# rahulgaur104/ideal-ballooning-solver

Measured on AMD Instinct MI355X. Metric: field-line eigenvalue solves/sec (N_zeta=512), higher is better.
Workload: dtype f64; 1 GPU; configs[1] D3D-shape: 16 surfaces x 8 alpha x 8 theta0 = 1024 solves/step/GPU, N_zeta=512 (513 points), geometry-fed scan with fused per-surface argmax (one launch); nonconverged=0, ranks_in_collective=1

## Files before the change

### ideal-ballooning-solver_amd/csrc/ibs_group.hpp

```cpp
#pragma once
#include "ibs_wave.hpp"

namespace ibs {

template <int P>
struct Grp {
  static_assert(P == 16 || P == 32 || P == 64, "group size");
  static constexpr int G = 64 / P;

  template <typename T>
  __device__ __forceinline__ static T bcast_last(T v, int lane) {
    if constexpr (P == 64) return readlane_t(v, 63);
    else if constexpr (P == 32) { const T a = readlane_t(v, 31), b = readlane_t(v, 63); return lane < 32 ? a : b; }
    else return dpp_t<0x15F, 0xF>(v, v);
  }
  __device__ __forceinline__ static int bcast_last_i(int v, int lane) {
    if constexpr (P == 64) return readlane_i(v, 63);
    else if constexpr (P == 32) { const int a = readlane_i(v, 31), b = readlane_i(v, 63); return lane < 32 ? a : b; }
    else return dpp_i<0x15F, 0xF>(v, v);
  }
  template <typename T>
  __device__ __forceinline__ static T sum(T v, int lane) {
    v += dppz_t<0x111, 0xF>(v);
    v += dppz_t<0x112, 0xF>(v);
// ... 56 lines not shown
    const int l16 = lane & 15, row = lane >> 4;
    { const M2<T> F = dpp_fetch<T, 0x101, 0xF>(Q); if (l16 < 15) Q = mul<T, false>(Q, F); }
    { const M2<T> F = dpp_fetch<T, 0x102, 0xF>(Q); if (l16 < 14) Q = mul<T, true>(Q, F); }
    { const M2<T> F = dpp_fetch<T, 0x104, 0xF>(Q); if (l16 < 12) Q = mul<T, false>(Q, F); }
    { const M2<T> F = dpp_fetch<T, 0x108, 0xF>(Q); if (l16 < 8) Q = mul<T, true>(Q, F); }
    if constexpr (P >= 32) {
      const M2<T> t16 = lane_bcast(Q, 16), t48 = lane_bcast(Q, 48);
      M2<T> F;
      F.a = row == 0 ? t16.a : t48.a; F.b = row == 0 ? t16.b : t48.b;
      F.c = row == 0 ? t16.c : t48.c; F.d = row == 0 ? t16.d : t48.d; F.e = row == 0 ? t16.e : t48.e;
      if ((row & 1) == 0) Q = mul<T, P == 32>(Q, F);
    }
    if constexpr (P == 64) { const M2<T> F = lane_bcast(Q, 32); if (row < 2) Q = mul<T, true>(Q, F); }
    return Q;
  }
};

template <typename T, int M, int P>
struct GroupSolver {
  using GP = Grp<P>;
  static constexpr int G = 64 / P;
  T D[M], Ph[M];
  T kap, ikap;
  bool has_last;
  int lane, lg, gid;
  T sig_vec;
  T zw[M];
  T u0_in;
  T zu_m1, zw_p1;
  int Eu, Ew;
  T lo, hi, normA;
  T trial_rho, trial_del;
  T trial_mrg;
  T shoot_m; int shoot_e;
  T fu, fw;
  int thr;

  __device__ __forceinline__ static int rows_start(int lg_, int n) {
    const int rem = n - P * (M - 1);
    return lg_ * (M - 1) + (lg_ < rem ? lg_ : rem);
  }

  template <class Src, bool TRIAL = false>
  __device__ __forceinline__ bool setup(const Src& src, int N, T h) {
    lane = threadIdx.x & 63;
    lg = lane & (P - 1);
    gid = lane / P;
    const int n = N - 2;
    const int rem = n - P * (M - 1);
    has_last = lg < rem;
    const int a = rows_start(lg, n);
    const T ih2 = T(1) / (h * h);
    T sc = T(1);
    const T g0 = src.g(a);
    T gcur = src.g(a + 1);
    T e_lo = T(0.5) * (g0 + gcur) * ih2;
    T vhi = -T(1e300), vlo = -T(1e300), vna = T(0), sum_c = T(0), sum_f = T(0);
    bool bad = !(g0 > T(0)) || !(gcur > T(0));
    const T e_first = e_lo;
    T ts_prev = T(0), ts_cur = T(0), two_cd = T(0), tA = T(0), tB = T(0), tC = T(0);
    if constexpr (TRIAL) {
      const T dl = T(3.14159265358979323846) / T(N - 1);
      T s0, c0, sd, cd;
      trial_sincos(T(a) * dl, s0, c0);
      trial_sincos(dl, sd, cd);
      ts_prev = s0; ts_cur = xfma(s0, cd, c0 * sd); two_cd = T(2) * cd;
    }
#pragma unroll
    for (int i = 0; i < M; ++i) {
      const bool act = (i < M - 1) || has_last;
      if (act) {
        const int j = a + i + 1;
        const T gnext = src.g(j + 1);
        bad = bad || !(gnext > T(0));
        const T e_hi = T(0.5) * (gcur + gnext) * ih2;
        const T cj = src.c(j), fj = src.f(j);
        const T d = cj - (e_lo + e_hi);
        const T s2 = sc * sc;
        D[i] = d * s2; Ph[i] = fj * s2;
        const T rf = fast_rcp(fj);
        if constexpr (TRIAL) {
          const T ts_next = xfma(two_cd, ts_cur, -ts_prev);
          const T Tx = xfma(e_lo, ts_prev, xfma(d, ts_cur, e_hi * ts_next));
          tA = xfma(ts_cur, Tx, tA); tB = xfma(fj * ts_cur, ts_cur, tB); tC = xfma(Tx * rf, Tx, tC);
          ts_prev = ts_cur; ts_cur = ts_next;
        }
        vhi = xmax(vhi, cj * rf);
        vlo = xmax(vlo, d * rf);
        vna = xmax(vna, (xabs(d) + e_lo + e_hi) * rf);
        sum_c += cj; sum_f += fj;
        bad = bad || !(fj > T(0)) || !(e_hi > T(0)) || !finite_of(cj);
        sc = fast_rcp(e_hi * sc);
        gcur = gnext; e_lo = e_hi;
      } else {
        D[i] = T(0); Ph[i] = T(0);
      }
    }
    kap = sc; ikap = fast_rcp(sc);
    bad = bad || !(e_first > T(0));
    const T ends = GP::sum((lg == 0 ? e_first : T(0)) + (lg == P - 1 ? e_lo : T(0)), lane);
    const T sc_all = GP::sum(sum_c, lane), sf_all = GP::sum(sum_f, lane);
    normA = GP::max(vna, lane);
    hi = GP::max(vhi, lane);
    lo = xmax(GP::max(vlo, lane), (sc_all - ends) / sf_all);
    hi += T(8) * Eps<T>::v * normA;
    lo -= T(8) * Eps<T>::v * normA;
    if constexpr (TRIAL) {
      const T A = GP::sum(tA, lane), B = GP::sum(tB, lane), C = GP::sum(tC, lane);
      const T rho = A / B;
      trial_rho = rho;
      trial_del = approx_sqrt(xmax(xfma(-rho, A, C), T(0)) / B);
    } else {
      trial_rho = T(0); trial_del = T(-1);
    }
    trial_mrg = T(8 + N / 2) * Eps<T>::v * normA;
    chk_slack = T(N < 256 ? 2 * N : 512) * Eps<T>::v * normA;
    return GP::sum_i(bad ? 1 : 0, lane) != 0;
  }

  __device__ __forceinline__ void trial_guess(bool take, T& guess, T& width, bool& warm) {
    const bool use = take && finite_of(trial_rho) && trial_del > T(0) && trial_del < T(0.25) * (hi - lo);
    lo = use ? xmax(lo, trial_rho - trial_mrg) : lo;
    guess = use ? trial_rho : guess;
    width = use ? T(0.25) * trial_del : width;
    warm = use ? true : warm;
  }

  template <bool STORE = true>
// ... 108 lines not shown
      const T a_um1 = readlane_t(zum_b, sLk), a_wp1 = readlane_t(zwp_b, sLk);
      const int a_ik = readlane_i(bi, sLk), a_Eu = readlane_i(Eu, sLk), a_Ew = readlane_i(Ew, sLk);
      zu_k = mine ? a_zu : zu_k; zw_k = mine ? a_zw : zw_k; t_k = mine ? a_t : t_k;
      um1 = mine ? a_um1 : um1; wp1 = mine ? a_wp1 : wp1;
      ik = mine ? a_ik : ik; Euk = mine ? a_Eu : Euk; Ewk = mine ? a_Ew : Ewk;
    }
    const T uw = zu_k * zw_k;
    const T num = xfma(um1, zw_k, xfma(t_k, uw, wp1 * zu_k));
    int du = Eu - Euk, dw = Ew - Ewk;
    du = du > 1000 ? 1000 : (du < -2000 ? -2000 : du);
    dw = dw > 1000 ? 1000 : (dw < -2000 ? -2000 : dw);
    fu = xldexp(fast_rcp(zu_k), du);
    fw = xldexp(fast_rcp(zw_k), dw);
    thr = (lane < Lk) ? M : ((lane > Lk) ? -1 : ik);
    T acc = T(0);
    static_assert(M + 2 <= 32, "sign word");
    unsigned su = sign_word(zu_m1) >> 31, sw = 0;
    {
      T zc = u0_in, zp = zu_m1;
#pragma unroll
      for (int i = 0; i < M; ++i) {
        const T t = xfma(-sig, Ph[i], D[i]);
        const bool act = (i < M - 1) || has_last;
        const T xu = zc * fu, xw = zw[i] * fw;
        const T x = (i <= thr) ? xu : xw;
        if (act) acc = xfma(Ph[i] * x, x, acc);
        if constexpr (CNT) {
          su = (unsigned)__builtin_amdgcn_alignbit(su, sign_word(zc), 31);
          sw = (unsigned)__builtin_amdgcn_alignbit(sw, sign_word(zw[i]), 31);
        }
        const T zn = xfma(-t, zc, -zp);
        if (act) { zp = zc; zc = zn; }
      }
    }
    if constexpr (CNT) {
      const int last = has_last ? M - 1 : M - 2;
      const int iu = thr < last ? thr : last;
      const unsigned mu = iu >= 0 ? (((1u << (iu + 1)) - 1u) << (M - 1 - iu)) : 0u;
      const int iw = thr > 0 ? thr : 0;
      const unsigned mw = iw <= last ? (((1u << (last - iw + 1)) - 1u) << (M - last)) : 0u;
      const unsigned sw2 = (sw << 1) | (sign_word(zw_p1) >> 31);
      extra_above = GP::sum_i(__builtin_popcount((su ^ (su >> 1)) & mu) + __builtin_popcount((sw2 ^ (sw2 << 1)) & mw), lane);
    }
    sig_vec = sig;
    const T tot = GP::sum(acc, lane);
    return sig + num * fast_rcp(uw * tot);
  }

  template <class Src>
  __device__ __forceinline__ void assemble(const Src& src, int N, T h, T (&x)[M]) {
    const int a = rows_start(lg, N - 2);
    const T ih2 = T(1) / (h * h);
    T sc = T(1);
    T gcur = src.g(a + 1);
    T zc = u0_in, zp = zu_m1;
#pragma unroll
    for (int i = 0; i < M; ++i) {
      const bool act = (i < M - 1) || has_last;
      const T xu = sc * zc * fu, xw = sc * zw[i] * fw;
      x[i] = act ? ((i <= thr) ? xu : xw) : T(0);
      if (act) {
        const T gnext = src.g(a + i + 2);
        sc = fast_rcp(T(0.5) * (gcur + gnext) * ih2 * sc);
        gcur = gnext;
        const T zn = xfma(-xfma(-sig_vec, Ph[i], D[i]), zc, -zp);
        zp = zc; zc = zn;
      }
    }
  }

  bool suspect, closed;
  T rho_last;
  __device__ __forceinline__ int why() const {
    const T tol = T(64) * Eps<T>::v * normA, rho = rho_last;
    const T dist = xmax(xmax(lo - rho, rho - hi), T(0));
    int bk = dist > T(0) ? expo_of(dist) - expo_of(tol) + 8 : 0;
    bk = finite_of(rho) ? (bk < 1 ? (dist > T(0) ? 1 : 0) : (bk > 63 ? 63 : bk)) : 63;
    return closed ? (bk | (extra_above != 0 ? 64 : 0)) : 0;
  }
  T chk_slack;
  template <bool CHK = false>
  __device__ __forceinline__ T solve(bool bad, int& iters_out, int& status_out, bool warm = false, T guess = T(0),
                                     T width = T(0)) {
    using WS = WaveSolver<T, M>;
    using Pt = typename WS::Pt;
    const T tol = (sizeof(T) == 8 ? T(64) : T(8)) * Eps<T>::v * normA;
    const bool warm_ok = warm && finite_of(guess) && width > T(0) && guess + width < hi && guess + width > lo;
    bool expand = warm_ok, try_below = warm_ok;
    T wstep = T(4) * width;
    const T g_below = guess - width;
    T sig = warm_ok ? guess + width : T(0.5) * (lo + hi), sig_prev = sig, lam = hi;
    T off_up = tol, off_dn = tol, rho_trust = hi;
    int aimed = 0, it = 0, lg_prev = 0;
    bool lo1 = false, hi_f = false, old_ok = false, was_interp = false, conv = false;
    Pt Plo{lo, T(0), 0}, Phi{hi, T(0), 0}, Pold{hi, T(0), 0};
    bool done = bad;
    constexpr int kMaxIt = 200;
    int guard = 0;
    auto sel = [](bool c, const Pt& a, const Pt& b) { return Pt{c ? a.x : b.x, c ? a.m : b.m, c ? a.e : b.e}; };
    while (__any(!done) && guard < kMaxIt) {
      ++guard;
      const int C = sweep_fwd<true>(sig);
      const bool act = !done;
      it += act ? 1 : 0;
      const Pt cur{sig, shoot_m, shoot_e};
      const bool uh = act && C == 0, ul = act && C != 0;
      const bool t1 = uh && hi_f, t2 = ul && lo1;
      Pold = sel(t1, Phi, sel(t2, Plo, Pold)); old_ok = old_ok || t1 || t2;
      hi = uh ? sig : hi; Phi = sel(uh, cur, Phi); hi_f = hi_f || uh;
      lo = ul ? sig : lo; Plo = sel(ul, cur, Plo); lo1 = ul ? (C == 1) : lo1;
      const T prevstep = xabs(sig - sig_prev);
      sig_prev = sig;
      const int e_now = expo_of(shoot_m);
      const int red = lg_prev - (e_now < -(1 << 27) ? e_now : shoot_e + e_now);
      conv = was_interp ? (red >= 4) : (aimed != 0 ? conv : false);
      const bool force_bis = was_interp && red < 1;
      const bool cert = aimed != 0;
// ... 75 lines not shown
```

### ideal-ballooning-solver_amd/csrc/ibs_kernels.hip

```cpp
#include "ibs_wave.hpp"
#include "ibs_launch.hpp"
#include "ibs_refine.hpp"
#include <type_traits>

#ifndef IBS_M
#error "compile with -DIBS_M=<rows per lane>"
#endif
#ifndef IBS_DIRECT_MIN_M
#define IBS_DIRECT_MIN_M 9
#endif
#ifndef IBS_F32LAM_DIRECT_MIN_M
#define IBS_F32LAM_DIRECT_MIN_M 3
#endif

namespace ibs {

template <typename T>
struct SrcGCF {
  static constexpr bool kHasGh = false;
  const T* gs; const T* cs; const T* fs;
  __device__ __forceinline__ T g(int j) const { return gs[lpos(j)]; }
  __device__ __forceinline__ T c(int j) const { return cs[lpos(j)]; }
  __device__ __forceinline__ T f(int j) const { return fs[lpos(j)]; }
  __device__ __forceinline__ void gcf(int j, T& g_, T& c_, T& f_) const { const int q = lpos(j); g_ = gs[q]; c_ = cs[q]; f_ = fs[q]; }
// ... 139 lines not shown
      src.gcf(jc, g_, c_, f_);
    }
    y0 += c_ * X2 - g_ * dX2;
    y1 = xfma(f_, X2, y1);
    if constexpr (!std::is_same<Tan, NoTangent>::value) {
      T ga, ca, fa;
      tan->at(jc, ga, ca, fa);
      ac = xfma(ca, X2, ac); ag = xfma(ga, dX2, ag); af = xfma(fa, X2, af);
    }
    if (X_out && in) X_out[sys * N + j] = (TO)X;
    if (dX_out && in) dX_out[sys * N + j] = (TO)dX;
  }
  IBS_PROBE_AT(14);
  y0 = wave_sum(y0); y1 = wave_sum(y1);
  const T gam = y0 / y1;
  if constexpr (HF) {
    if (do_hf) {
      hc = wave_sum(hc); hg = wave_sum(hg); hf = wave_sum(hf);
      const T jac = hc / y1 - hg / y1 - gam * hf / y1;
      if (lane == 0) dth0_out[sys] = (TO)jac;
    }
  }
  if constexpr (!std::is_same<Tan, NoTangent>::value) {
    ac = wave_sum(ac); ag = wave_sum(ag); af = wave_sum(af);
    const T jac = ac / y1 - ag / y1 - gam * af / y1;
    if (lane == 0 && dalpha_out) dalpha_out[sys] = (TO)jac;
  }
  if (lane == 0) {
    if (gam_out) __hip_atomic_store(gam_out + sys, (TO)gam, __ATOMIC_RELAXED, __HIP_MEMORY_SCOPE_AGENT);
    if (lam_out) lam_out[sys] = (TO)lam;
    if (info_out) info_out[sys] = inf.iters | (inf.status << 16);
  }
}

template <typename T, class Src, bool WT>
__device__ __forceinline__ void simpson_point(const Src& src, int j, T w, T X, T dX, T& y0, T& y1, T& hc, T& hg, T& hf) {
  const T X2 = w * (X * X), dX2 = w * (dX * dX);
  T g_, c_, f_;
  if constexpr (WT) {
    T gt, ct, ft;
    src.gcf_with_tangent(j, g_, c_, f_, gt, ct, ft);
    hc = xfma(ct, X2, hc); hg = xfma(gt, dX2, hg); hf = xfma(ft, X2, hf);
  } else {
    src.gcf(j, g_, c_, f_);
  }
  y0 += c_ * X2 - g_ * dX2;
  y1 = xfma(f_, X2, y1);
}

template <typename T, class Src, bool WT>
__device__ __forceinline__ void simpson_point_carried(const Src& src, int j, T a1, T d_, T c_, T f_, T w, T X, T dX, T& y0, T& y1,
                                                      T& hc, T& hg, T& hf) {
  const T X2 = w * (X * X), dX2 = w * (dX * dX);
  asm volatile("" : "+v"(d_));
  const T g_ = a1 * d_;
  if constexpr (WT) {
    T gt, ct, ft;
    src.tangent(j, a1, gt, ct, ft);
    hc = xfma(ct, X2, hc); hg = xfma(gt, dX2, hg); hf = xfma(ft, X2, hf);
  }
  y0 += c_ * X2 - g_ * dX2;
  y1 = xfma(f_, X2, y1);
}

template <typename T, int M, class Src, bool HF, int PASSES = 1, typename TO = T, bool RES = false>
__device__ __forceinline__ void finish_chunk(WaveSolver<T, M, RES>& ws, Src& src, int N, T h, T* Xs, T lam,
                                             const SolveInfo& inf, long sys, typename TypeId<TO>::type* lam_out,
                                             typename TypeId<TO>::type* gam_out, typename TypeId<TO>::type* X_out,
                                             typename TypeId<TO>::type* dX_out, typename TypeId<TO>::type* dth0_out,
                                             int* info_out, const T* gh = nullptr) {
  static_assert(M >= 3, "the halo exchange takes two rows from each neighbour lane");
  const int lane = ws.lane;
  const int n = N - 2;
  const bool hl = ws.has_last;
  T x[M];
  ws.assemble(src, gh, N, h, x);
  T m = T(0);
#pragma unroll
  for (int i = 0; i < M; ++i) m = xmax(m, xabs(x[i]));
  m = uniform(wave_max(m));
  const T rm = T(1) / m;
#pragma unroll
  for (int i = 0; i < M; ++i) x[i] *= rm;
  int a = WaveSolver<T, M>::rows_start(lane, n);
  asm volatile("" : "+v"(a));
  const T lastv = hl ? x[M - 1] : x[M - 2], last2 = hl ? x[M - 2] : x[M - 3];
  const T xp1 = dpp_t<0x130, 0xF>(T(0), x[0]), xp2 = dpp_t<0x130, 0xF>(T(0), x[1]);
  T xe[M + 4];
  xe[0] = dpp_t<0x138, 0xF>(T(0), last2); xe[1] = dpp_t<0x138, 0xF>(T(0), lastv);
#pragma unroll
  for (int i = 0; i < M - 1; ++i) xe[i + 2] = x[i];
  xe[M + 1] = hl ? x[M - 1] : xp1; xe[M + 2] = hl ? xp1 : xp2; xe[M + 3] = xp2;
  IBS_PROBE_AT(13);
  T ih;
  if constexpr (RES) ih = ws.rr.ih; else ih = T(1) / h;
  const T A_in = (T(2) / T(3)) * ih, B_in = -ih / T(12), A_e1 = T(0.5) * ih, A_e0 = T(2) * ih, B_e0 = T(-0.5) * ih;
  bool do_hf = false;
  if constexpr (HF) do_hf = dth0_out != nullptr;
  T y0 = T(0), y1 = T(0), hc = T(0), hg = T(0), hf = T(0);
  const T w_even = ((a + 1) & 1) ? T(4) : T(2), w_odd = ((a + 1) & 1) ? T(2) : T(4);
  const int i_end = (lane == kWave - 1) ? (hl ? M - 1 : M - 2) : -1;
  const T dX_end = xfma(A_e0, lane == 0 ? x[0] : -lastv, B_e0 * (lane == 0 ? x[1] : -last2));
  auto all_points = [&](auto with_tangent) {
    if (lane == 0 || lane == kWave - 1)
      simpson_point<T, Src, HF && decltype(with_tangent)::value>(src, lane == 0 ? 0 : N - 1, T(1), T(0), dX_end, y0, y1, hc, hg, hf);
#pragma unroll
    for (int i = 0; i < M; ++i) {
// ... 1545 lines not shown
```

### ideal-ballooning-solver_amd/csrc/ibs_kernels_group.hip

```cpp
#include <type_traits>
#include "ibs_group.hpp"
#include "ibs_launch.hpp"

#if !defined(IBS_M) || !defined(IBS_P)
#error "compile with -DIBS_P=<lanes per system> -DIBS_M=<rows per lane>"
#endif

namespace ibs {

template <typename T, typename TI = T>
struct SrcGlobal {
  static constexpr bool kHasGh = false;
  const TI* gs; const TI* cs; const TI* fs;
  __device__ __forceinline__ T g(int j) const { return (T)gs[j]; }
  __device__ __forceinline__ T c(int j) const { return (T)cs[j]; }
  __device__ __forceinline__ T f(int j) const { return (T)fs[j]; }
};

template <typename T>
struct SrcGeoG {
  static constexpr bool kHasGh = false;
  const T* A1; const T* A3; const T* C0; const T* C1; const T* G0; const T* G1; const T* G2;
  T th0, two_th0, th0sq;
  __device__ __forceinline__ T gd(int j) const { const int q = lpos(j); return G0[q] + two_th0 * G1[q] + th0sq * G2[q]; }
  __device__ __forceinline__ T g(int j) const { return A1[lpos(j)] * gd(j); }
  __device__ __forceinline__ T c(int j) const { const int q = lpos(j); return C0[q] + th0 * C1[q]; }
  __device__ __forceinline__ T f(int j) const { return A3[lpos(j)] * gd(j); }
  __device__ __forceinline__ T gdp(int j) const { const int q = lpos(j); return T(2) * G1[q] + two_th0 * G2[q]; }
  __device__ __forceinline__ T g_t(int j) const { return A1[lpos(j)] * gdp(j); }
  __device__ __forceinline__ T c_t(int j) const { return C1[lpos(j)]; }
  __device__ __forceinline__ T f_t(int j) const { return A3[lpos(j)] * gdp(j); }
};

template <typename T, class Src, bool WT>
__device__ __forceinline__ void simpson_point_g(const Src& src, int j, T w, T X, T dX, T& y0, T& y1, T& hc, T& hg, T& hf) {
  const T X2 = w * (X * X), dX2 = w * (dX * dX);
  y0 += src.c(j) * X2 - src.g(j) * dX2;
  y1 = xfma(src.f(j), X2, y1);
  if constexpr (WT) { hc = xfma(src.c_t(j), X2, hc); hg = xfma(src.g_t(j), dX2, hg); hf = xfma(src.f_t(j), X2, hf); }
}

template <typename T, int M, int P, class Src, bool HF, typename TO = T>
__device__ __forceinline__ void finish_chunk_g(GroupSolver<T, M, P>& ws, const Src& src, int N, T h, T* Xs, T lam,
                                               int iters, int status, long sys, bool valid, TO* lam_out, TO* gam_out,
                                               TO* X_out, TO* dX_out, TO* dth0_out, int* info_out) {
  static_assert(M >= 3, "the halo exchange takes two rows from each neighbour lane");
  using GP = Grp<P>;
  const int lane = ws.lane, lg = ws.lg;
  const int n = N - 2;
  const bool hl = ws.has_last, first = lg == 0, last = lg == P - 1;

  T x[M];
  ws.assemble(src, N, h, x);
  T m = T(0);
#pragma unroll
  for (int i = 0; i < M; ++i) m = xmax(m, xabs(x[i]));
  m = GP::max(m, lane);
  const T rm = T(1) / m;
#pragma unroll
  for (int i = 0; i < M; ++i) x[i] *= rm;
  int a = GroupSolver<T, M, P>::rows_start(lg, n);
  asm volatile("" : "+v"(a));
  const T lastv = hl ? x[M - 1] : x[M - 2], last2 = hl ? x[M - 2] : x[M - 3];
  const T sp1 = dpp_t<0x130, 0xF>(T(0), x[0]), sp2 = dpp_t<0x130, 0xF>(T(0), x[1]);
  const T sm2 = dpp_t<0x138, 0xF>(T(0), last2), sm1 = dpp_t<0x138, 0xF>(T(0), lastv);
  const T xp1 = last ? T(0) : sp1, xp2 = last ? T(0) : sp2;
  T xe[M + 4];
  xe[0] = first ? T(0) : sm2; xe[1] = first ? T(0) : sm1;
#pragma unroll
  for (int i = 0; i < M - 1; ++i) xe[i + 2] = x[i];
  xe[M + 1] = hl ? x[M - 1] : xp1; xe[M + 2] = hl ? xp1 : xp2; xe[M + 3] = xp2;
  const T ih = T(1) / h;
  const T A_in = (T(2) / T(3)) * ih, B_in = -ih / T(12), A_e1 = T(0.5) * ih, A_e0 = T(2) * ih, B_e0 = T(-0.5) * ih;
  bool do_hf = false;
  if constexpr (HF) do_hf = dth0_out != nullptr;
  T y0 = T(0), y1 = T(0), hc = T(0), hg = T(0), hf = T(0);
  const T w_even = ((a + 1) & 1) ? T(4) : T(2), w_odd = ((a + 1) & 1) ? T(2) : T(4);
  const int i_end = last ? (hl ? M - 1 : M - 2) : -1;
// ... 310 lines not shown
```

### ideal-ballooning-solver_amd/csrc/ibs_wave.hpp

```cpp
#pragma once
#include <hip/hip_runtime.h>
#include <type_traits>
#include "ibs_sweep_count.hpp"

namespace ibs {

constexpr int kWave = 64;

#ifdef IBS_TRACE_ALL
__device__ double ibs_trace_all[404];
#endif
#ifdef IBS_PROBE
__device__ long long ibs_probe_buf[(16 + 4) * 4096];
#define IBS_PROBE_SLOT(k) ibs_probe_buf[(k) < 16 ? (blockIdx.x * 4 + (threadIdx.x >> 6)) * 16 + (k) \
                                                 : 16 * 4096 + (blockIdx.x * 4 + (threadIdx.x >> 6)) * 4 + ((k) - 16)]
#define IBS_PROBE_NOW() wall_clock64()
#define IBS_PROBE_PUT(k, t) do { if ((threadIdx.x & 63) == 0 && blockIdx.x < 1024 && threadIdx.x < 256) IBS_PROBE_SLOT(k) = (t); } while (0)
#define IBS_PROBE_AT(k) IBS_PROBE_PUT(k, wall_clock64())
#else
#define IBS_PROBE_AT(k) do {} while (0)
#define IBS_PROBE_NOW() 0LL
#define IBS_PROBE_PUT(k, t) do { (void)(t); } while (0)
#endif



__device__ __forceinline__ int fexp(double x) { return __builtin_amdgcn_frexp_exp(x); }
__device__ __forceinline__ int fexp(float x) { return __builtin_amdgcn_frexp_expf(x); }
__device__ __forceinline__ double xldexp(double x, int e) { return __builtin_ldexp(x, e); }
__device__ __forceinline__ float xldexp(float x, int e) { return __builtin_ldexpf(x, e); }
__device__ __forceinline__ double xfma(double a, double b, double c) { return __builtin_fma(a, b, c); }
__device__ __forceinline__ float xfma(float a, float b, float c) { return __builtin_fmaf(a, b, c); }
__device__ __forceinline__ double xabs(double a) { return __builtin_fabs(a); }
__device__ __forceinline__ float xabs(float a) { return __builtin_fabsf(a); }
__device__ __forceinline__ double xmax(double a, double b) { return __builtin_fmax(a, b); }
__device__ __forceinline__ float xmax(float a, float b) { return __builtin_fmaxf(a, b); }
__device__ __forceinline__ double xmin(double a, double b) { return __builtin_fmin(a, b); }
__device__ __forceinline__ float xmin(float a, float b) { return __builtin_fminf(a, b); }
__device__ __forceinline__ bool signbit_of(double a) { return __double2hiint(a) < 0; }
__device__ __forceinline__ bool signbit_of(float a) { return __float_as_int(a) < 0; }
__device__ __forceinline__ bool sign_differs(double a, double b) {
  int x = __double2hiint(a) ^ __double2hiint(b);
  asm("" : "+v"(x));
  return x < 0;
}
__device__ __forceinline__ bool sign_differs(float a, float b) { return (__float_as_int(a) ^ __float_as_int(b)) < 0; }
__device__ __forceinline__ unsigned sign_word(double a) { return (unsigned)__double2hiint(a); }
__device__ __forceinline__ unsigned sign_word(float a) { return (unsigned)__float_as_int(a); }
__device__ __forceinline__ bool finite_of(double a) { return xabs(a) <= 1.7976931348623157e308; }
__device__ __forceinline__ bool finite_of(float a) { return xabs(a) <= 3.4028234e38f; }

__device__ __forceinline__ double fast_rcp(double x) {
  double r = __builtin_amdgcn_rcp(x);
  r = __builtin_fma(__builtin_fma(-x, r, 1.0), r, r);
  r = __builtin_fma(__builtin_fma(-x, r, 1.0), r, r);
  return r;
// ... 317 lines not shown
}

template <typename T, class CountF>
__device__ __forceinline__ bool multisect(CountF&& count, T lo, T hi, T normA, T stop_eps, int lane, T& lam, int& passes) {
  const T epsA = Eps<T>::v * normA;
  bool ok = false;
  passes = 0;
  while (passes < 24) {
    ++passes;
    const T w = hi - lo;
    const T sig = lane == kWave - 1 ? hi : xfma(T(lane) * T(1.0 / 63.0), w, lo);
    const int cnt = count(sig);
    const unsigned long long m = __builtin_amdgcn_ballot_w64(cnt >= 1);
    if (!(m & 1ull)) { hi = lo; lo = lo - T(64) * w; continue; }
    const int top = 63 - __builtin_clzll(m);
    if (top == kWave - 1) { lo = hi; hi = hi + T(64) * w; continue; }
    lo = readlane_t(sig, top); hi = readlane_t(sig, top + 1);
    if (!(hi - lo > stop_eps * epsA)) { ok = true; break; }
  }
  lam = T(0.5) * (lo + hi);
  return ok;
}
template <typename T, class CountF>
__device__ __forceinline__ bool multisect_k(CountF&& count, int k, T lo, T hi, T normA, T stop_eps, int lane, T& lam, int& passes) {
  const T epsA = Eps<T>::v * normA;
  bool ok = false;
  passes = 0;
  while (passes < 24) {
    ++passes;
    const T w = hi - lo;
    const T sig = lane == kWave - 1 ? hi : xfma(T(lane) * T(1.0 / 63.0), w, lo);
    const int cnt = count(sig);
    const unsigned long long m = __builtin_amdgcn_ballot_w64(cnt >= k);
    if (!(m & 1ull)) { hi = lo; lo = lo - T(64) * w; continue; }
    const int top = 63 - __builtin_clzll(m);
    if (top == kWave - 1) { lo = hi; hi = hi + T(64) * w; continue; }
    lo = readlane_t(sig, top); hi = readlane_t(sig, top + 1);
    if (!(hi - lo > stop_eps * epsA)) { ok = true; break; }
  }
  lam = T(0.5) * (lo + hi);
  return ok;
}
template <typename T, class Src>
__device__ __forceinline__ bool multisect_division(const Src& src, int N, T h, T lo, T hi, T normA, int lane, T& lam, int& passes) {
  const T ih2 = T(1) / (h * h);
  return multisect<T>([&](T sig) { return count_above_div<T, Src>(src, N, ih2, sig); }, lo, hi, normA, T(2), lane, lam, passes);
}
template <typename T, class Src>
__device__ __forceinline__ bool reclose_division(const Src& src, int N, T h, T center, T normA, int lane, T& lam, int& passes) {
  const T epsA = Eps<T>::v * normA;
  return multisect_division<T, Src>(src, N, h, center - T(2048) * epsA, center + T(2048) * epsA, normA, lane, lam, passes);
}

struct SolveInfo {
  int iters;
  int status;
};

template <typename T, int M, bool RES>
struct ResidentRows {};
template <typename T, int M>
struct ResidentRows<T, M, true> {
  T a1[M], d[M], c[M], f[M], zu[M];
  T ih2, ih;
  unsigned own;
};

template <typename T, int M, bool RES = false>
struct WaveSolver {
  ResidentRows<T, M, RES> rr;
  T D[M], Ph[M];
  T kap, ikap;
  bool has_last;
  int lane;
  T zw[M];
  T u0_in, zu_m1;
  T zw_p1;
  int Eu, Ew;
  T sig_vec;
  T lo, hi, normA;
  T trial_rho, trial_del;
  T trial_mrg;
  T shoot_m; int shoot_e;

  static constexpr int kSetupRows = 4;
  __device__ __forceinline__ static int rows_start(int lane, int n) {
    const int rem = n - kWave * (M - 1);
    return lane * (M - 1) + (lane < rem ? lane : rem);
  }

  template <class Src, bool TRIAL = false>
  __device__ __forceinline__ bool setup(const Src& src, int N, T h) {
    lane = threadIdx.x & (kWave - 1);
    const int n = N - 2;
    const int rem = n - kWave * (M - 1);
    has_last = lane < rem;
    if constexpr (RES) rr.own = sweep_count_mask(M, has_last, lane == kWave - 1);
    const int a = rows_start(lane, n);
    T ih2;
    if constexpr (RES) ih2 = rr.ih2; else ih2 = T(1) / (h * h);
    T sc = T(1);
    T gcur = T(0);
    T e_lo;
    bool bad = false;
    if constexpr (Src::kHasGh) {
      e_lo = src.gh(a) * ih2;
      bad = !(src.g(a) > T(0));
    } else {
      const T g0 = src.g(a);
      gcur = src.g(a + 1);
      e_lo = T(0.5) * (g0 + gcur) * ih2;
      bad = !(g0 > T(0)) || !(gcur > T(0));
    }
    T vhi = -T(1e300), vlo = -T(1e300), vna = T(0), sum_c = T(0), sum_f = T(0);
    const T e_first = e_lo;
    T ts_prev = T(0), ts_cur = T(0), two_cd = T(0), tA = T(0), tB = T(0), tC = T(0);
    if constexpr (TRIAL) {
      const T dl = T(3.14159265358979323846) / T(N - 1);
      T s0, c0, sd, cd;
      trial_sincos(T(a) * dl, s0, c0);
      trial_sincos(dl, sd, cd);
      ts_prev = s0; ts_cur = xfma(s0, cd, c0 * sd); two_cd = T(2) * cd;
    }
#pragma unroll
    for (int i = 0; i < M; ++i) {
      const bool act = (i < M - 1) || has_last;
      if (act) {
        const int j = a + i + 1;
        T gnext = T(0), e_hi;
        if constexpr (Src::kHasGh) { e_hi = src.gh(j) * ih2; bad = bad || !(src.g(j + 1) > T(0)); }
        else { gnext = src.g(j + 1); e_hi = T(0.5) * (gcur + gnext) * ih2; bad = bad || !(gnext > T(0)); }
        const T cj = src.c(j), fj = src.f(j);
        const T d = cj - (e_lo + e_hi);
        const T s2 = sc * sc;
        D[i] = d * s2; Ph[i] = fj * s2;
        const T rf = fast_rcp(fj);
        if constexpr (TRIAL) {
          const T ts_next = xfma(two_cd, ts_cur, -ts_prev);
          const T Tx = xfma(e_lo, ts_prev, xfma(d, ts_cur, e_hi * ts_next));
          tA = xfma(ts_cur, Tx, tA); tB = xfma(fj * ts_cur, ts_cur, tB); tC = xfma(Tx * rf, Tx, tC);
          ts_prev = ts_cur; ts_cur = ts_next;
        }
        vhi = xmax(vhi, cj * rf);
        vlo = xmax(vlo, d * rf);
        vna = xmax(vna, (xabs(d) + e_lo + e_hi) * rf);
        sum_c += cj; sum_f += fj;
        bad = bad || !(fj > T(0)) || !(e_hi > T(0)) || !finite_of(cj);
        if constexpr (RES) { src.g_factors(j, rr.a1[i], rr.d[i]); rr.c[i] = cj; rr.f[i] = fj; }
        sc = fast_rcp(e_hi * sc);
        gcur = gnext; e_lo = e_hi;
      } else {
        D[i] = T(0); Ph[i] = T(0);
        if constexpr (RES) { rr.a1[i] = T(0); rr.d[i] = T(0); rr.c[i] = T(0); rr.f[i] = T(0); }
      }
      if constexpr (M > 8) { if ((i % kSetupRows) == kSetupRows - 1) __builtin_amdgcn_sched_barrier(0); }
    }
    IBS_PROBE_AT(8);
    kap = sc; ikap = fast_rcp(sc);
    bad = bad || !(e_first > T(0));
    const T e0 = readlane_t(e_first, 0);
    const T en = readlane_t(e_lo, kWave - 1);
    const T sc_all = wave_sum(sum_c), sf_all = wave_sum(sum_f);
    normA = uniform(wave_max(vna));
    hi = uniform(wave_max(vhi));
    lo = uniform(xmax(wave_max(vlo), (sc_all - e0 - en) / sf_all));
    hi += T(8) * Eps<T>::v * normA;
    lo -= T(8) * Eps<T>::v * normA;
    if constexpr (TRIAL) {
      const T A = wave_sum(tA), B = wave_sum(tB), C = wave_sum(tC);
      const T rho = A / B;
      trial_rho = rho;
      trial_del = approx_sqrt(xmax(xfma(-rho, A, C), T(0)) / B);
    } else {
      trial_rho = T(0); trial_del = T(-1);
    }
    trial_mrg = T(8 + N / 2) * Eps<T>::v * normA;
    chk_slack = T(N < 256 ? 2 * N : 512) * Eps<T>::v * normA;
    IBS_PROBE_AT(9);
    return __any(bad) != 0;
  }

  __device__ __forceinline__ void trial_guess(T& guess, T& width) {
    const bool use = U(finite_of(trial_rho) && trial_del > T(0) && trial_del < T(0.25) * (hi - lo));
    if (use) lo = xmax(lo, trial_rho - trial_mrg);
    guess = use ? trial_rho : T(__builtin_nanf(""));
    width = T(0.25) * trial_del;
  }

  __device__ __forceinline__ int sweep_fwd(T sig) {
    T fA = T(1), fAp = T(0), fB = T(0), fBp = T(1);
#pragma unroll
    for (int i = 0; i < M; ++i) {
      const T tf = xfma(-sig, Ph[i], D[i]);
      if ((i < M - 1) || has_last) {
        const T nA = xfma(-tf, fA, -fAp), nB = xfma(-tf, fB, -fBp);
        fAp = fA; fA = nA; fBp = fB; fB = nB;
      }
    }
    M2<T> F;
    F.a = fA * kap; F.b = fB * kap; F.c = fAp * ikap; F.d = fBp * ikap; F.e = 0;
    renorm(F);
    const M2<T> P = scan_fwd(F, lane);
    shoot_m = readlane_t(P.a, kWave - 1); shoot_e = readlane_i(P.e, kWave - 1);
    const T u0 = dpp_t<0x138, 0xF>(T(1), P.a);
    const T um = dpp_t<0x138, 0xF>(T(0), P.c);
    Eu = dpp_i<0x138, 0xF>(0, P.e);
// ... 147 lines not shown
    unsigned su_b = 0, sw_a = 0, sw_b = 0, su_a = sign_word(zu_m1) >> 31;
    {
      T zc = u0_in, zp = zu_m1;
#pragma unroll
      for (int i = 0; i < M; ++i) {
        const bool act = (i < M - 1) || has_last;
        if constexpr (RES) zc = rr.zu[i];
        const T xu = zc * fu, xw = zw[i] * fw;
        const T x = (i <= thr) ? xu : xw;
        if (act) acc = xfma(Ph[i] * x, x, acc);
        if constexpr (CNT) {
          if constexpr (sizeof(SignWord) == 4) {
            su = (unsigned)__builtin_amdgcn_alignbit(su, sign_word(zc), 31);
            sw = (unsigned)__builtin_amdgcn_alignbit(sw, sign_word(zw[i]), 31);
          } else if (i < MH) {
            su_a = (unsigned)__builtin_amdgcn_alignbit(su_a, sign_word(zc), 31);
            sw_a = (unsigned)__builtin_amdgcn_alignbit(sw_a, sign_word(zw[i]), 31);
          } else {
            su_b = (unsigned)__builtin_amdgcn_alignbit(su_b, sign_word(zc), 31);
            sw_b = (unsigned)__builtin_amdgcn_alignbit(sw_b, sign_word(zw[i]), 31);
          }
        }
        if constexpr (!RES) {
          const T zn = xfma(-xfma(-sig, Ph[i], D[i]), zc, -zp);
          if (act) { zp = zc; zc = zn; }
        }
      }
    }
    if constexpr (CNT) {
      if constexpr (sizeof(SignWord) == 8) {
        su = ((SignWord)su_a << (M - MH)) | (SignWord)su_b;
        sw = ((SignWord)sw_a << (M - MH)) | (SignWord)sw_b;
      }
      const int last = has_last ? M - 1 : M - 2;
      const int iu = thr < last ? thr : last;
      const SignWord one = 1;
      const SignWord mu = iu >= 0 ? (((one << (iu + 1)) - one) << (M - 1 - iu)) : SignWord(0);
      const int iw = thr > 0 ? thr : 0;
      const SignWord mw = iw <= last ? (((one << (last - iw + 1)) - one) << (M - last)) : SignWord(0);
      const SignWord sw2 = (sw << 1) | (SignWord)(sign_word(zw_p1) >> 31);
      const SignWord fl_u = (su ^ (su >> 1)) & mu, fl_w = (sw2 ^ (sw2 << 1)) & mw;
      int c;
      if constexpr (sizeof(SignWord) == 4) c = __builtin_popcount(fl_u) + __builtin_popcount(fl_w);
      else c = __builtin_popcountll(fl_u) + __builtin_popcountll(fl_w);
      extra_above = wave_sum_i(c);
    }
    sig_vec = sig;
    const T tot = wave_sum(acc);
    return sig + num * fast_rcp(uw * tot);
  }

  template <class Src>
  __device__ __forceinline__ void assemble(const Src& src, const T* gh, int N, T h, T (&x)[M]) {
    int a = rows_start(lane, N - 2);
    asm volatile("" : "+v"(a));
    T ih2;
    if constexpr (RES) ih2 = rr.ih2; else ih2 = T(1) / (h * h);
    T sc = T(1);
    T gcur = src.g(a + 1);
    T zc = u0_in, zp = zu_m1;
#pragma unroll
    for (int i = 0; i < M; ++i) {
      const bool act = (i < M - 1) || has_last;
      if constexpr (RES) zc = rr.zu[i];
      const T xu = sc * zc * fu, xw = sc * zw[i] * fw;
      x[i] = act ? ((i <= thr) ? xu : xw) : T(0);
      if (act) {
        T e_hi;
        if (gh) e_hi = gh[a + i + 1] * ih2;
        else { const T gnext = src.g(a + i + 2); e_hi = T(0.5) * (gcur + gnext) * ih2; gcur = gnext; }
        sc = fast_rcp(e_hi * sc);
        if constexpr (!RES) {
          const T zn = xfma(-xfma(-sig_vec, Ph[i], D[i]), zc, -zp);
          zp = zc; zc = zn;
        }
      }
      if ((i & 3) == 3) __builtin_amdgcn_sched_barrier(0);
    }
  }

#ifdef IBS_TRACE
  T* trace = nullptr;
#endif
#ifdef IBS_TRACE_ALL
#define IBS_TRACE_SWEEP(it_, sig_, C_, lo_, hi_) do { if (sizeof(T) == 8 && blockIdx.x == 0 && threadIdx.x == 0 && (it_) <= 100) { \
    double* q_ = ibs_trace_all + 4 * ((it_) - 1); q_[0] = (double)(sig_); q_[1] = (double)(C_); q_[2] = (double)(lo_); q_[3] = (double)(hi_); ibs_trace_all[400] = (double)(it_); } } while (0)
#else
#define IBS_TRACE_SWEEP(it_, sig_, C_, lo_, hi_) do {} while (0)
#endif
  struct Pt { T x, m; int e; };
  __device__ __forceinline__ static bool U(bool c) { return __builtin_amdgcn_ballot_w64(c) != 0ull; }
  __device__ __forceinline__ static int uniform_i(int v) { return __builtin_amdgcn_readfirstlane(v); }
  __device__ __forceinline__ static int lg2_of(const Pt& p) { const int e = expo_of(p.m); return e < -(1 << 27) ? e : p.e + e; }
  __device__ __forceinline__ static bool interpolate(const Pt& o, bool use_o, const Pt& a, const Pt& b,
                                                     T lo_, T hi_, T& rho) {
    constexpr int L = ExpLim<T>::v;
    int emax = a.e > b.e ? a.e : b.e;
    if (use_o && o.e > emax) emax = o.e;
    auto val = [&](const Pt& p) { int d = p.e - emax; d = d < -L ? -L : d; return p.m * pow2_of<T>(d); };
    const T x2 = b.x, f1 = val(a), f2 = val(b), f0 = val(o);
    const T h2r = x2 - a.x;
    int k = expo_of(h2r);
    k = k < -L ? -L : (k > L ? L : k);
    const T sc = pow2_of<T>(-k), back = pow2_of<T>(k);
    const T h2 = h2r * sc, h1 = (a.x - o.x) * sc;
    const T df21 = f2 - f1;
    const T z_s = -f2 * h2 * approx_rcp(df21);
    const T r_s = xfma(z_s, back, x2);
    const bool in_s = finite_of(r_s) && r_s > lo_ && r_s < hi_;
    const T S = h1 + h2;
    const T QA = xfma(df21, h1, -(f1 - f0) * h2);
    const T QB = xfma(QA, h2, df21 * h1 * S);
    const T H = h1 * h2 * S;
    const T disc = xfma(QB, QB, -T(4) * QA * f2 * H);
    const T sq = approx_sqrt(xmax(disc, T(0)));
    const T den = QB >= T(0) ? QB + sq : QB - sq;
    const T z1 = -T(2) * f2 * H * approx_rcp(den);
    const T z2 = -den * approx_rcp(T(2) * QA);
    const T r1 = xfma(z1, back, x2), r2 = xfma(z2, back, x2);
    const bool par = use_o && disc >= T(0) && H != T(0);
    const bool in1 = par && finite_of(r1) && r1 > lo_ && r1 < hi_;
    const bool in2 = par && finite_of(r2) && r2 > lo_ && r2 < hi_;
    const bool pick1 = in1 && (!in2 || xabs(z1) <= xabs(z2));
    rho = pick1 ? r1 : (in2 ? r2 : r_s);
    return in1 || in2 || in_s;
  }
  __device__ __forceinline__ static bool interpolate_lazy(const Pt& o, bool use_o, const Pt& a, const Pt& b,
                                                          T lo_, T hi_, bool need, T& rho) {
// ... 206 lines not shown
```

Baseline: 45.81 million solves/s.

## Carry half-grid g factors across rows and cache per-row scales in resident rows

Adds a HalfGridWalk helper that loads the A1 and gd factors for each grid point once and carries them to the next row. The half-grid mean is then formed with a fixed fused-multiply-add ordering, so each g value is no longer reloaded and recomputed twice per row. In resident mode the setup pass also stores the per-row similarity scale s[i], letting assemble skip recomputing the reciprocal chain and reading geometry. The cost is M extra registers per lane for s[], which may raise register pressure and lower occupancy, and the changed rounding order may alter results slightly.

New measurement: 47.14 million solves/s, median of 6. 1.03x the previous value.

```diff
diff --git a/ideal-ballooning-solver_amd/csrc/ibs_group.hpp b/ideal-ballooning-solver_amd/csrc/ibs_group.hpp
--- a/ideal-ballooning-solver_amd/csrc/ibs_group.hpp
+++ b/ideal-ballooning-solver_amd/csrc/ibs_group.hpp
@@ -132,9 +132,11 @@
     const int a = rows_start(lg, n);
     const T ih2 = T(1) / (h * h);
     T sc = T(1);
-    const T g0 = src.g(a);
-    T gcur = src.g(a + 1);
-    T e_lo = T(0.5) * (g0 + gcur) * ih2;
+    constexpr bool kWalk = HalfGridWalk<T, Src, M>::kFactors;
+    HalfGridWalk<T, Src, M> hg;
+    T g0, gcur, e_lo;
+    if constexpr (kWalk) { hg.begin(src, a); g0 = hg.g; e_lo = hg.next(src, 0, a) * ih2; gcur = hg.g; }
+    else { g0 = src.g(a); gcur = src.g(a + 1); e_lo = T(0.5) * (g0 + gcur) * ih2; }
     T vhi = -T(1e300), vlo = -T(1e300), vna = T(0), sum_c = T(0), sum_f = T(0);
     bool bad = !(g0 > T(0)) || !(gcur > T(0));
     const T e_first = e_lo;
@@ -151,9 +153,9 @@
       const bool act = (i < M - 1) || has_last;
       if (act) {
         const int j = a + i + 1;
-        const T gnext = src.g(j + 1);
-        bad = bad || !(gnext > T(0));
-        const T e_hi = T(0.5) * (gcur + gnext) * ih2;
+        T gnext, e_hi;
+        if constexpr (kWalk) { e_hi = hg.next(src, i + 1, j) * ih2; gnext = hg.g; bad = bad || !(gnext > T(0)); }
+        else { gnext = src.g(j + 1); bad = bad || !(gnext > T(0)); e_hi = T(0.5) * (gcur + gnext) * ih2; }
         const T cj = src.c(j), fj = src.f(j);
         const T d = cj - (e_lo + e_hi);
         const T s2 = sc * sc;
@@ -368,7 +370,10 @@
     const int a = rows_start(lg, N - 2);
     const T ih2 = T(1) / (h * h);
     T sc = T(1);
-    T gcur = src.g(a + 1);
+    constexpr bool kWalk = HalfGridWalk<T, Src, M>::kFactors;
+    HalfGridWalk<T, Src, M> hg;
+    T gcur = T(0);
+    if constexpr (kWalk) hg.begin(src, a + 1); else gcur = src.g(a + 1);
     T zc = u0_in, zp = zu_m1;
 #pragma unroll
     for (int i = 0; i < M; ++i) {
@@ -376,9 +381,14 @@
       const T xu = sc * zc * fu, xw = sc * zw[i] * fw;
       x[i] = act ? ((i <= thr) ? xu : xw) : T(0);
       if (act) {
-        const T gnext = src.g(a + i + 2);
-        sc = fast_rcp(T(0.5) * (gcur + gnext) * ih2 * sc);
-        gcur = gnext;
+        if constexpr (kWalk) {
+          const T e_hi = hg.next(src, i + 1, a + i + 1) * ih2;
+          sc = fast_rcp(e_hi * sc);
+        } else {
+          const T gnext = src.g(a + i + 2);
+          sc = fast_rcp(T(0.5) * (gcur + gnext) * ih2 * sc);
+          gcur = gnext;
+        }
         const T zn = xfma(-xfma(-sig_vec, Ph[i], D[i]), zc, -zp);
         zp = zc; zc = zn;
       }
diff --git a/ideal-ballooning-solver_amd/csrc/ibs_half_grid.hpp b/ideal-ballooning-solver_amd/csrc/ibs_half_grid.hpp
--- /dev/null
+++ b/ideal-ballooning-solver_amd/csrc/ibs_half_grid.hpp
@@ -0,0 +1,50 @@
+#pragma once
+
+#if defined(__HIPCC__) || defined(__CUDACC__)
+#define IBS_HG_HD __host__ __device__ __attribute__((always_inline))
+#else
+#define IBS_HG_HD __attribute__((always_inline))
+#endif
+
+namespace ibs {
+
+IBS_HG_HD inline double half_grid_fma(double a, double b, double c) { return __builtin_fma(a, b, c); }
+IBS_HG_HD inline float half_grid_fma(float a, float b, float c) { return __builtin_fmaf(a, b, c); }
+
+IBS_HG_HD constexpr bool half_grid_fuses_lower(int k, int M) { return k == 0 || ((k ^ M) & 1) != 0; }
+
+template <typename T>
+IBS_HG_HD inline T half_grid_product(T a1, T d) {
+#pragma clang fp contract(off)
+  return a1 * d;
+}
+
+template <typename T>
+IBS_HG_HD inline T half_grid_mean_fused(T a1_f, T d_f, T g_r) {
+#pragma clang fp contract(off)
+  return T(0.5) * half_grid_fma(a1_f, d_f, g_r);
+}
+
+template <typename T>
+IBS_HG_HD inline T half_grid_mean(int k, int M, T a1_lo, T d_lo, T a1_hi, T d_hi) {
+  return half_grid_fuses_lower(k, M) ? half_grid_mean_fused(a1_lo, d_lo, half_grid_product(a1_hi, d_hi))
+                                  : half_grid_mean_fused(a1_hi, d_hi, half_grid_product(a1_lo, d_lo));
+}
+
+template <typename T>
+IBS_HG_HD inline T half_grid_mean_plain(T g_lo, T g_hi) {
+#pragma clang fp contract(off)
+  return T(0.5) * (g_lo + g_hi);
+}
+
+template <typename T>
+IBS_HG_HD inline T half_grid_scale(T mean, T ih2) {
+#pragma clang fp contract(off)
+  return mean * ih2;
+}
+template <typename T>
+IBS_HG_HD inline T half_grid_e(int k, int M, T a1_lo, T d_lo, T a1_hi, T d_hi, T ih2) {
+  return half_grid_scale(half_grid_mean(k, M, a1_lo, d_lo, a1_hi, d_hi), ih2);
+}
+
+}
diff --git a/ideal-ballooning-solver_amd/csrc/ibs_kernels.hip b/ideal-ballooning-solver_amd/csrc/ibs_kernels.hip
--- a/ideal-ballooning-solver_amd/csrc/ibs_kernels.hip
+++ b/ideal-ballooning-solver_amd/csrc/ibs_kernels.hip
@@ -215,7 +215,6 @@
 __device__ __forceinline__ void simpson_point_carried(const Src& src, int j, T a1, T d_, T c_, T f_, T w, T X, T dX, T& y0, T& y1,
                                                       T& hc, T& hg, T& hf) {
   const T X2 = w * (X * X), dX2 = w * (dX * dX);
-  asm volatile("" : "+v"(d_));
   const T g_ = a1 * d_;
   if constexpr (WT) {
     T gt, ct, ft;
diff --git a/ideal-ballooning-solver_amd/csrc/ibs_kernels_group.hip b/ideal-ballooning-solver_amd/csrc/ibs_kernels_group.hip
--- a/ideal-ballooning-solver_amd/csrc/ibs_kernels_group.hip
+++ b/ideal-ballooning-solver_amd/csrc/ibs_kernels_group.hip
@@ -24,6 +24,7 @@
   T th0, two_th0, th0sq;
   __device__ __forceinline__ T gd(int j) const { const int q = lpos(j); return G0[q] + two_th0 * G1[q] + th0sq * G2[q]; }
   __device__ __forceinline__ T g(int j) const { return A1[lpos(j)] * gd(j); }
+  __device__ __forceinline__ void g_factors(int j, T& a1, T& d_) const { a1 = A1[lpos(j)]; d_ = gd(j); }
   __device__ __forceinline__ T c(int j) const { const int q = lpos(j); return C0[q] + th0 * C1[q]; }
   __device__ __forceinline__ T f(int j) const { return A3[lpos(j)] * gd(j); }
   __device__ __forceinline__ T gdp(int j) const { const int q = lpos(j); return T(2) * G1[q] + two_th0 * G2[q]; }
diff --git a/ideal-ballooning-solver_amd/csrc/ibs_wave.hpp b/ideal-ballooning-solver_amd/csrc/ibs_wave.hpp
--- a/ideal-ballooning-solver_amd/csrc/ibs_wave.hpp
+++ b/ideal-ballooning-solver_amd/csrc/ibs_wave.hpp
@@ -2,6 +2,7 @@
 #include <hip/hip_runtime.h>
 #include <type_traits>
 #include "ibs_sweep_count.hpp"
+#include "ibs_half_grid.hpp"
 
 namespace ibs {
 
@@ -425,6 +426,30 @@
   return multisect_division<T, Src>(src, N, h, center - T(2048) * epsA, center + T(2048) * epsA, normA, lane, lam, passes);
 }
 
+template <class Src, typename T, typename = void>
+struct SrcHasGFactors : std::false_type {};
+template <class Src, typename T>
+struct SrcHasGFactors<Src, T, std::void_t<decltype(std::declval<const Src&>().g_factors(0, std::declval<T&>(), std::declval<T&>()))>>
+    : std::true_type {};
+
+template <typename T, class Src, int M>
+struct HalfGridWalk {
+  static constexpr bool kFactors = SrcHasGFactors<Src, T>::value;
+  T a1, d;
+  T g;
+  __device__ __forceinline__ void load(const Src& src, int j, T& a1_, T& d_, T& g_) const {
+    src.g_factors(j, a1_, d_); g_ = half_grid_product(a1_, d_);
+  }
+  __device__ __forceinline__ void begin(const Src& src, int j) { load(src, j, a1, d, g); }
+  __device__ __forceinline__ T next(const Src& src, int k, int j) {
+    T a1n, dn, gn;
+    load(src, j + 1, a1n, dn, gn);
+    const T m = half_grid_fuses_lower(k, M) ? half_grid_mean_fused(a1, d, gn) : half_grid_mean_fused(a1n, dn, g);
+    a1 = a1n; d = dn; g = gn;
+    return m;
+  }
+};
+
 struct SolveInfo {
   int iters;
   int status;
@@ -434,7 +459,7 @@
 struct ResidentRows {};
 template <typename T, int M>
 struct ResidentRows<T, M, true> {
-  T a1[M], d[M], c[M], f[M], zu[M];
+  T a1[M], d[M], c[M], f[M], zu[M], s[M];
   T ih2, ih;
   unsigned own;
 };
@@ -473,12 +498,19 @@
     T ih2;
     if constexpr (RES) ih2 = rr.ih2; else ih2 = T(1) / (h * h);
     T sc = T(1);
+    constexpr bool kWalk = HalfGridWalk<T, Src, M>::kFactors;
+    HalfGridWalk<T, Src, M> hg;
     T gcur = T(0);
     T e_lo;
     bool bad = false;
     if constexpr (Src::kHasGh) {
       e_lo = src.gh(a) * ih2;
       bad = !(src.g(a) > T(0));
+    } else if constexpr (kWalk) {
+      hg.begin(src, a);
+      const T g0 = hg.g;
+      e_lo = hg.next(src, 0, a) * ih2;
+      bad = !(g0 > T(0)) || !(hg.g > T(0));
     } else {
       const T g0 = src.g(a);
       gcur = src.g(a + 1);
@@ -501,7 +533,9 @@
       if (act) {
         const int j = a + i + 1;
         T gnext = T(0), e_hi;
+        if constexpr (RES) { rr.a1[i] = hg.a1; rr.d[i] = hg.d; rr.s[i] = sc; }
         if constexpr (Src::kHasGh) { e_hi = src.gh(j) * ih2; bad = bad || !(src.g(j + 1) > T(0)); }
+        else if constexpr (kWalk) { e_hi = hg.next(src, i + 1, j) * ih2; bad = bad || !(hg.g > T(0)); }
         else { gnext = src.g(j + 1); e_hi = T(0.5) * (gcur + gnext) * ih2; bad = bad || !(gnext > T(0)); }
         const T cj = src.c(j), fj = src.f(j);
         const T d = cj - (e_lo + e_hi);
@@ -519,12 +553,12 @@
         vna = xmax(vna, (xabs(d) + e_lo + e_hi) * rf);
         sum_c += cj; sum_f += fj;
         bad = bad || !(fj > T(0)) || !(e_hi > T(0)) || !finite_of(cj);
-        if constexpr (RES) { src.g_factors(j, rr.a1[i], rr.d[i]); rr.c[i] = cj; rr.f[i] = fj; }
+        if constexpr (RES) { rr.c[i] = cj; rr.f[i] = fj; }
         sc = fast_rcp(e_hi * sc);
         gcur = gnext; e_lo = e_hi;
       } else {
         D[i] = T(0); Ph[i] = T(0);
-        if constexpr (RES) { rr.a1[i] = T(0); rr.d[i] = T(0); rr.c[i] = T(0); rr.f[i] = T(0); }
+        if constexpr (RES) { rr.a1[i] = T(0); rr.d[i] = T(0); rr.c[i] = T(0); rr.f[i] = T(0); rr.s[i] = T(0); }
       }
       if constexpr (M > 8) { if ((i % kSetupRows) == kSetupRows - 1) __builtin_amdgcn_sched_barrier(0); }
     }
@@ -778,28 +812,37 @@
 
   template <class Src>
   __device__ __forceinline__ void assemble(const Src& src, const T* gh, int N, T h, T (&x)[M]) {
+    if constexpr (RES) {
+#pragma unroll
+      for (int i = 0; i < M; ++i) {
+        const bool act = (i < M - 1) || has_last;
+        const T xu = rr.s[i] * rr.zu[i] * fu, xw = rr.s[i] * zw[i] * fw;
+        x[i] = act ? ((i <= thr) ? xu : xw) : T(0);
+      }
+      return;
+    }
     int a = rows_start(lane, N - 2);
     asm volatile("" : "+v"(a));
-    T ih2;
-    if constexpr (RES) ih2 = rr.ih2; else ih2 = T(1) / (h * h);
+    const T ih2 = T(1) / (h * h);
     T sc = T(1);
-    T gcur = src.g(a + 1);
+    constexpr bool kWalk = HalfGridWalk<T, Src, M>::kFactors;
+    HalfGridWalk<T, Src, M> hg;
+    T gcur = T(0);
+    if constexpr (kWalk) hg.begin(src, a + 1); else gcur = src.g(a + 1);
     T zc = u0_in, zp = zu_m1;
 #pragma unroll
     for (int i = 0; i < M; ++i) {
       const bool act = (i < M - 1) || has_last;
-      if constexpr (RES) zc = rr.zu[i];
       const T xu = sc * zc * fu, xw = sc * zw[i] * fw;
       x[i] = act ? ((i <= thr) ? xu : xw) : T(0);
       if (act) {
         T e_hi;
         if (gh) e_hi = gh[a + i + 1] * ih2;
+        else if constexpr (kWalk) e_hi = hg.next(src, i + 1, a + i + 1) * ih2;
         else { const T gnext = src.g(a + i + 2); e_hi = T(0.5) * (gcur + gnext) * ih2; gcur = gnext; }
         sc = fast_rcp(e_hi * sc);
-        if constexpr (!RES) {
-          const T zn = xfma(-xfma(-sig_vec, Ph[i], D[i]), zc, -zp);
-          zp = zc; zc = zn;
-        }
+        const T zn = xfma(-xfma(-sig_vec, Ph[i], D[i]), zc, -zp);
+        zp = zc; zc = zn;
       }
       if ((i & 3) == 3) __builtin_amdgcn_sched_barrier(0);
     }
```
